# fragarriss/CurVis

Measured on AMD Instinct MI355X. Metric: Mrays/s (pixels x steps/s) at 1920x1080, 4096 steps, higher is better.
Workload: dtype f64

## Files before the change

curvis_amd/csrc/cv_sampler_dev.h:

```cpp
#ifndef CURVIS_CV_SAMPLER_DEV_H
#define CURVIS_CV_SAMPLER_DEV_H

#include "cv_math.h"

#if defined(__clang__)
#pragma clang fp contract(off)
#endif

namespace cvk {

constexpr unsigned kSamplerCap = 1536;
constexpr unsigned kSamplerPendCap = 1024;

enum : int { SAMPLER_OK = 0, SAMPLER_PANIC = 1, SAMPLER_OVERFLOW = 2 };

struct SamplerResult {
  unsigned n, rounds;
  unsigned long long calls, steps;
  int warned, status;
  unsigned eval_phases, evaluated;
};

constexpr unsigned kSpecSlots = 8192;
constexpr unsigned kSpecEvalCap = 2048;
constexpr unsigned kSpecEvalSoft = 1024;
constexpr unsigned long long kSpecEmpty = ~0ull;

struct SpecTable {
  unsigned long long *key;
  double *e, *s;
  unsigned *steps;
  int *status;
};

#if defined(__HIP_DEVICE_COMPILE__)
#define CV_SPEC_CAS(p, expect, val) atomicCAS((p), (expect), (val))
#define CV_SPEC_LD(p) __hip_atomic_load((p), __ATOMIC_RELAXED, __HIP_MEMORY_SCOPE_AGENT)
#define CV_SPEC_ST(p, v) __hip_atomic_store((p), (v), __ATOMIC_RELAXED, __HIP_MEMORY_SCOPE_AGENT)
#else
static inline unsigned long long cv_spec_cas_host(unsigned long long *p, unsigned long long expect, unsigned long long val) {
  const unsigned long long old = *p;
  if (old == expect) *p = val;
  return old;
}
#define CV_SPEC_CAS(p, expect, val) cv_spec_cas_host((p), (expect), (val))
#define CV_SPEC_LD(p) (*(p))
#define CV_SPEC_ST(p, v) (*(p) = (v))
#endif

CV_HD unsigned long long spec_key(double a) {
  unsigned long long k;
  __builtin_memcpy(&k, &a, sizeof k);
  return k;
}
CV_HD unsigned spec_hash(unsigned long long k) { return (unsigned)((k * 0x9E3779B97F4A7C15ull) >> 44) & (kSpecSlots - 1u); }
CV_HD unsigned spec_claim(const SpecTable &T, unsigned long long k, bool &fresh) {
  unsigned i = spec_hash(k);
  for (;;) {
    const unsigned long long old = CV_SPEC_CAS(&T.key[i], kSpecEmpty, k);
    if (old == kSpecEmpty) {
      fresh = true;
      return i;
    }
    if (old == k) {
      fresh = false;
      return i;
    }
    i = (i + 1u) & (kSpecSlots - 1u);
  }
}
CV_HD int spec_find(const SpecTable &T, unsigned long long k) {
  unsigned i = spec_hash(k);
  for (;;) {
    const unsigned long long cur = CV_SPEC_LD(&T.key[i]);
    if (cur == k) return (int)i;
    if (cur == kSpecEmpty) return -1;
    i = (i + 1u) & (kSpecSlots - 1u);
  }
}

CV_HD bool sampler_refine(double a1, double e1, double s1, double a2, double e2, double s2, double a3, double e3, double s3,
                          double thr1, double thr2) {
  const double area1 = CV_FABS((a1 * e2 + a2 * e3 + a3 * e1) - (e1 * a2 + e2 * a3 + e3 * a1));
  const double area2 = CV_FABS((a1 * s2 + a2 * s3 + a3 * s1) - (s1 * a2 + s2 * a3 + s3 * a1));
  return area1 > thr1 || area2 > thr2;
}
CV_HD bool sampler_finite(double v) { return (v - v) == 0.0; }

struct SamplerState {
  double a[2][kSamplerCap], e[2][kSamplerCap], s[2][kSamplerCap];
  double pend_a[kSamplerPendCap];
  unsigned short pend_out[kSamplerPendCap];
  unsigned char flag[kSamplerCap];
  unsigned short vis[kSamplerCap], vis_out[kSamplerCap];
  unsigned cur, n, n_new, n_pend, n_vis, iteration, prev_amount, rounds;
  int started, finished, panicked, warned, overflow, go, nonfinite;
  unsigned long long calls, steps;
  unsigned short miss[kSamplerPendCap];
  double eval_a[kSpecEvalCap];
  unsigned short eval_slot[kSpecEvalCap];
  unsigned n_miss, n_eval, n_cached , eval_phases, evaluated;
};

CV_HD void sampler_reset(SamplerState &S) {
  S.cur = S.n = S.n_new = S.n_pend = S.n_vis = S.iteration = S.prev_amount = S.rounds = 0u;
  S.started = S.finished = S.panicked = S.warned = S.overflow = S.go = S.nonfinite = 0;
  S.calls = S.steps = 0ull;
  S.n_miss = S.n_eval = S.n_cached = S.eval_phases = S.evaluated = 0u;
}


#if defined(__HIP_DEVICE_COMPILE__)
#define CV_LDS_INC(p) atomicAdd((p), 1u)
#define CV_LDS_ADD64(p, v) atomicAdd((p), (unsigned long long)(v))
#else
#define CV_LDS_INC(p) ((*(p))++)
#define CV_LDS_ADD64(p, v) (*(p) += (unsigned long long)(v))
#endif
struct SamplerState;
CV_HD void sampler_store(SamplerState &S, unsigned t, double e, double s);

CV_HD void sampler_finish(SamplerState &S, unsigned max_iterations) {
  if (S.iteration == max_iterations) S.warned = 1;
  S.finished = 1;
}

enum : int { PLAN_STOP = 0, PLAN_GRID = 1, PLAN_REFINE = 2 };

CV_HD int sampler_plan_begin(SamplerState &S, unsigned n0, unsigned max_iterations) {
  S.n_pend = 0u;
  if (S.finished) return PLAN_STOP;
  if (!S.started) {
    if (n0 > kSamplerCap || n0 > kSamplerPendCap) {
      S.overflow = S.finished = 1;
      return PLAN_STOP;
    }
    S.n_pend = S.n_new = n0;
    return PLAN_GRID;
  }
  if (!(S.iteration < max_iterations)) {
    sampler_finish(S, max_iterations);
    return PLAN_STOP;
  }
  S.prev_amount = S.n;
  if (S.n < 3u) {
    S.panicked = S.finished = 1;
    return PLAN_STOP;
  }
  return PLAN_REFINE;
}
CV_HD void sampler_grid_point(SamplerState &S, unsigned i, unsigned n0, double a_min, double a_max) {
  const double step = (a_max - a_min) / (double)(n0 - 1u);
  S.pend_a[i] = a_min + (double)i * step;
  S.pend_out[i] = (unsigned short)i;
}
CV_HD void sampler_flag(SamplerState &S, unsigned i, double thr1, double thr2) {
  const double *A = S.a[S.cur], *E = S.e[S.cur], *Z = S.s[S.cur];
  S.flag[i] = sampler_refine(A[i], E[i], Z[i], A[i + 1u], E[i + 1u], Z[i + 1u], A[i + 2u], E[i + 2u], Z[i + 2u], thr1, thr2) ? 1 : 0;
}
CV_HD bool sampler_walk(SamplerState &S) {
  const unsigned n = S.n;
  unsigned i = 0u, out = 0u, k = 0u, v = 0u;
  while (i < n - 2u) {
    if (out + 5u > kSamplerCap || k + 2u > kSamplerPendCap) {
      S.overflow = S.finished = 1;
      return false;
    }
    const unsigned f = S.flag[i];
    S.vis[v] = (unsigned short)(i | (f << 15));
    S.vis_out[v] = (unsigned short)out;
    ++v;
    if (f) {
      out += 4u, k += 2u, i += 2u;
    } else {
      out += 1u, i += 1u;
    }
  }
  S.n_vis = v;
  S.n_new = out;
  S.n_pend = k;
  return true;
}
CV_HD void sampler_place(SamplerState &S, unsigned v) {
  const unsigned dst = S.cur ^ 1u;
  const double *A = S.a[S.cur], *E = S.e[S.cur], *Z = S.s[S.cur];
  double *NA = S.a[dst], *NE = S.e[dst], *NZ = S.s[dst];
  const unsigned i = S.vis[v] & 0x7fffu, out = S.vis_out[v];
  NA[out] = A[i], NE[out] = E[i], NZ[out] = Z[i];
  if (S.vis[v] >> 15) {
    const unsigned k = 2u * ((out - v) / 3u);
    S.pend_a[k] = (A[i] + A[i + 1u]) / 2.0;
    S.pend_out[k] = (unsigned short)(out + 1u);
    NA[out + 2u] = A[i + 1u], NE[out + 2u] = E[i + 1u], NZ[out + 2u] = Z[i + 1u];
    S.pend_a[k + 1u] = (A[i + 1u] + A[i + 2u]) / 2.0;
    S.pend_out[k + 1u] = (unsigned short)(out + 3u);
    NA[out + 4u] = A[i + 2u], NE[out + 4u] = E[i + 2u], NZ[out + 4u] = Z[i + 2u];
  }
}
CV_HD bool sampler_plan(SamplerState &S, unsigned n0, unsigned max_iterations, double a_min, double a_max, double thr1, double thr2) {
  const int mode = sampler_plan_begin(S, n0, max_iterations);
  if (mode == PLAN_STOP) return false;
  if (mode == PLAN_GRID) {
    for (unsigned i = 0; i < n0; ++i) sampler_grid_point(S, i, n0, a_min, a_max);
    return true;
  }
  for (unsigned i = 0; i + 2u < S.n; ++i) sampler_flag(S, i, thr1, thr2);
  if (!sampler_walk(S)) return false;
  for (unsigned v = 0; v < S.n_vis; ++v) sampler_place(S, v);
  return true;
}

CV_HD void sampler_store(SamplerState &S, unsigned t, double e, double s) {
  const unsigned dst = S.cur ^ 1u, o = S.pend_out[t];
  S.a[dst][o] = S.pend_a[t];
  S.e[dst][o] = e;
  S.s[dst][o] = s;
  if (!(sampler_finite(e) && sampler_finite(s))) S.nonfinite = 1;
}

CV_HD bool sampler_take(SamplerState &S, const SpecTable &T, unsigned t, int &panic) {
  const int slot = spec_find(T, spec_key(S.pend_a[t]));
  if (slot < 0) return false;
  sampler_store(S, t, CV_SPEC_LD(&T.e[slot]), CV_SPEC_LD(&T.s[slot]));
  CV_LDS_ADD64(&S.steps, CV_SPEC_LD(&T.steps[slot]));
  if (CV_SPEC_LD(&T.status[slot]) == -2) panic = 1;
  return true;
}
CV_HD bool sampler_want(SamplerState &S, const SpecTable &T, double alpha, bool must) {
  if (!must && (S.n_cached >= kSpecSlots / 2u || S.n_eval >= kSpecEvalSoft)) return false;
  if (S.n_cached >= kSpecSlots - 1024u || S.n_eval >= kSpecEvalCap - 512u) {
    if (must) S.overflow = 1;
    return false;
  }
  bool fresh;
  const unsigned slot = spec_claim(T, spec_key(alpha), fresh);
  if (!fresh) return true;
  CV_LDS_INC(&S.n_cached);
  const unsigned k = CV_LDS_INC(&S.n_eval);
  S.eval_a[k] = alpha;
  S.eval_slot[k] = (unsigned short)slot;
  return true;
}
CV_HD void sampler_subtree(SamplerState &S, const SpecTable &T, double lo, double hi, unsigned depth) {
  if (depth > 7u) depth = 7u;
  for (unsigned level = 0u; level < depth; ++level)
    for (unsigned i = 0u; i < (1u << level); ++i) {
      double a = lo, b = hi, mid = (a + b) / 2.0;
      bool ok = mid > a && mid < b;
      for (unsigned bit = level; ok && bit-- > 0u;) {
        if ((i >> bit) & 1u)
          a = mid;
        else
          b = mid;
        mid = (a + b) / 2.0;
        ok = mid > a && mid < b;
      }
      if (ok && !sampler_want(S, T, mid, false)) return;
    }
}
CV_HD unsigned sampler_spec_depth(unsigned n, unsigned budget) {
  unsigned d = 0u;
  while (d < 7u && (unsigned long long)n * ((2ull << d) - 1ull) <= budget) ++d;
  return d;
}
CV_HD void sampler_speculate(SamplerState &S, const SpecTable &T, unsigned m, unsigned depth, unsigned grid_depth) {
  const unsigned t = S.miss[m];
  if (!S.started) {
    if (grid_depth && t + 1u < S.n_pend) sampler_subtree(S, T, S.pend_a[t], S.pend_a[t + 1u], grid_depth);
    return;
  }
  const unsigned dst = S.cur ^ 1u, o = S.pend_out[t];
  if (depth > 1u) {
    sampler_subtree(S, T, S.a[dst][o - 1u], S.pend_a[t], depth - 1u);
    sampler_subtree(S, T, S.pend_a[t], S.a[dst][o + 1u], depth - 1u);
  }
}

CV_HD void sampler_consume(SamplerState &S, unsigned max_iterations) {
  S.calls += S.n_pend;
  const unsigned dst = S.cur ^ 1u;
  double *NA = S.a[dst], *NE = S.e[dst], *NZ = S.s[dst];
  unsigned k = S.n_new;
  if (S.nonfinite) {
    k = 0u;
    for (unsigned i = 0; i < S.n_new; ++i)
      if (sampler_finite(NA[i]) && sampler_finite(NE[i]) && sampler_finite(NZ[i])) {
        if (k != i) NA[k] = NA[i], NE[k] = NE[i], NZ[k] = NZ[i];
        ++k;
      }
    S.nonfinite = 0;
  }
  S.n = k;
  S.cur = dst;
  if (!S.started) {
    S.started = 1;
    return;
  }
  S.rounds++;
  if (S.n <= S.prev_amount) {
    sampler_finish(S, max_iterations);
    return;
  }
  S.iteration += 1u;
}

}
#endif
```

curvis_amd/csrc/efficient_host.h:

```cpp
#pragma once

namespace {


struct EfficientCall {
  const curvis_metric *metric;
  const curvis_camera *cams;
  uint32_t n_frames, max_iter;
  double max_radius, delta;
  uint32_t alpha_nums, max_iterations_sampling;
  double thr1, thr2;
  uint32_t filter = 0;
  uint32_t ss = 1;
};

int eval_escape_batch(curvis_ctx *ctx, const curvis_metric *metric, const cvk::MetricParams &MP,
                      const std::vector<double> &alpha, const std::vector<double> &lcam, uint32_t max_iter,
                      double max_radius, double delta, std::vector<double> &angle, std::vector<double> &space,
                      std::vector<uint32_t> &steps, std::vector<int> &status, double *ms_acc) {
  const size_t n = alpha.size();
  angle.resize(n);
  space.resize(n);
  steps.resize(n);
  status.resize(n);
// ... 117 lines not shown
template <typename SampleMs>
void efficient_statistics(curvis_ctx *ctx, uint32_t n_frames, size_t npix, const FrameCounters &FC, SampleMs sample_ms, float pixel_ms,
                          curvis_stats *stats, std::chrono::steady_clock::time_point t_begin) {
  uint64_t tot[FC_N] = {0}, total_steps = 0;
  ctx->last_frame_stats.assign(n_frames, curvis_stats{});
  for (uint32_t f = 0; f < n_frames; ++f) {
    uint64_t fc[FC_N];
    sum_frame_counters(ctx->h_counters, FC.slots, f, fc);
    for (int k = 0; k < FC_N; ++k) tot[k] += fc[k];
    curvis_stats &fs = ctx->last_frame_stats[f];
    counts_to_stats(fc, fs);
    fs.rays = (uint64_t)npix;
    fs.steps = ctx->last_sampling_info[f].steps;
    total_steps += fs.steps;
    fs.integrate_ms = sample_ms / n_frames;
    fs.shade_ms = pixel_ms / n_frames;
    fs.kernel_ms = fs.integrate_ms + fs.shade_ms;
    fs.total_ms = fs.kernel_ms;
  }
  if (stats) {
    counts_to_stats(tot, *stats);
    stats->rays = (uint64_t)npix * n_frames;
    stats->steps = total_steps;
    stats->integrate_ms = sample_ms;
    stats->shade_ms = pixel_ms;
    stats->kernel_ms = sample_ms + pixel_ms;
    stats->total_ms = std::chrono::duration<double, std::milli>(std::chrono::steady_clock::now() - t_begin).count();
  }
}

constexpr int kSamplerFallback = 1;

curvis_ctx::SamplerKey make_sampler_key(const curvis_ctx *ctx, const EfficientCall &c) {
  curvis_ctx::SamplerKey k;
  k.metric = *c.metric;
  k.n_frames = c.n_frames;
  k.max_iter = c.max_iter;
  k.alpha_nums = c.alpha_nums;
  k.max_iterations_sampling = c.max_iterations_sampling;
  k.max_radius = c.max_radius, k.delta = c.delta, k.thr1 = c.thr1, k.thr2 = c.thr2;
  k.fast = ctx->fast_math != 0 ? 1 : 0;
  k.speculate = ctx->sampling_speculation != 0 ? 1 : 0;
  k.l_frame.resize(c.n_frames);
  for (uint32_t f = 0; f < c.n_frames; ++f) k.l_frame[f] = c.cams[f].pos[1];
  return k;
}
bool sampler_key_equal(const curvis_ctx::SamplerKey &a, const curvis_ctx::SamplerKey &b) {
  auto same = [](const double &x, const double &y) { return std::memcmp(&x, &y, sizeof(double)) == 0; };
  if (a.metric.kind != b.metric.kind || !same(a.metric.rho, b.metric.rho) || !same(a.metric.m, b.metric.m) || !same(a.metric.a, b.metric.a))
    return false;
  if (a.n_frames != b.n_frames || a.max_iter != b.max_iter || a.alpha_nums != b.alpha_nums ||
      a.max_iterations_sampling != b.max_iterations_sampling || a.fast != b.fast || a.speculate != b.speculate)
    return false;
  if (!same(a.max_radius, b.max_radius) || !same(a.delta, b.delta) || !same(a.thr1, b.thr1) || !same(a.thr2, b.thr2)) return false;
  return a.l_frame.size() == b.l_frame.size() &&
         std::memcmp(a.l_frame.data(), b.l_frame.data(), sizeof(double) * a.l_frame.size()) == 0;
}

int sampler_submit(curvis_ctx *ctx, unsigned slot, hipStream_t stream, const EfficientCall &c, const cvk::MetricParams &MP) {
  const curvis_camera *cams = c.cams;
  const uint32_t n_frames = c.n_frames;
  curvis_ctx::SamplerSlot &S = ctx->samp[slot];
  if (S.seq != 0 && S.done) HIP_TRY(ctx, hipEventSynchronize(S.done));
  if (ctx->dev_samples.valid && ctx->dev_samples.slot == slot) ctx->dev_samples.overwritten = true;
  S.valid = false;
  S.job_of_frame.assign(n_frames, 0u);
  S.l_job.clear();
  {
    std::map<uint64_t, unsigned> seen;
    for (uint32_t f = 0; f < n_frames; ++f) {
      uint64_t key;
      std::memcpy(&key, &cams[f].pos[1], sizeof key);
      auto it = seen.find(key);
      if (it == seen.end()) {
        it = seen.emplace(key, (unsigned)S.l_job.size()).first;
        S.l_job.push_back(cams[f].pos[1]);
      }
      S.job_of_frame[f] = it->second;
    }
  }
  const unsigned n_jobs = (unsigned)S.l_job.size();
  const size_t T = (size_t)n_jobs * cvk::kSamplerCap, SS = (size_t)n_jobs * cvk::kSpecSlots;
  size_t off = 0;
  auto carve = [&](size_t bytes) {
    const size_t o = off;
    off += (bytes + 255) & ~(size_t)255;
    return o;
  };
  const size_t o_jf = carve(sizeof(unsigned) * n_frames), o_to = carve(sizeof(unsigned) * n_frames), o_go = carve(sizeof(unsigned) * n_frames),
               o_l = carve(sizeof(double) * n_jobs);
  const size_t staged = off;
  S.o_tab_off = o_to;
  S.o_grid_off = o_go;
  S.o_grid = carve(sizeof(unsigned) * n_jobs * (cvk::kInterpGrid + 1u));
  S.o_tab_n = carve(sizeof(unsigned) * n_frames);
  S.o_res = carve(sizeof(cvk::SamplerResult) * n_jobs);
  for (size_t &o : S.o_tab) o = carve(sizeof(double) * T);
  const size_t o_sk = carve(sizeof(unsigned long long) * SS), o_se = carve(sizeof(double) * SS), o_ss = carve(sizeof(double) * SS),
               o_st = carve(sizeof(unsigned) * SS), o_su = carve(sizeof(int) * SS);
  int rc = S.d.reserve(ctx, off);
  if (rc) return rc;
  S.res_bytes = sizeof(cvk::SamplerResult) * n_jobs;
  S.h_res_off = staged;
  const size_t pinned = staged + ((S.res_bytes + 255) & ~(size_t)255);
  if ((rc = S.h.reserve(ctx, pinned, pinned / 2))) return rc;
  if ((rc = S.done.ensure(ctx, hipEventDisableTiming))) return rc;
  if ((rc = S.t0.ensure(ctx))) return rc;
  if ((rc = S.t1.ensure(ctx))) return rc;
  std::memcpy(S.h + o_jf, S.job_of_frame.data(), sizeof(unsigned) * n_frames);
  {
    auto *to = reinterpret_cast<unsigned *>(S.h + o_to);
    auto *go = reinterpret_cast<unsigned *>(S.h + o_go);
    for (uint32_t f = 0; f < n_frames; ++f) {
      to[f] = S.job_of_frame[f] * cvk::kSamplerCap;
      go[f] = S.job_of_frame[f] * (cvk::kInterpGrid + 1u);
    }
  }
  std::memcpy(S.h + o_l, S.l_job.data(), sizeof(double) * n_jobs);
  HIP_TRY(ctx, hipMemcpyAsync(S.d, S.h, staged, hipMemcpyHostToDevice, stream));
  HIP_TRY(ctx, hipMemsetAsync(S.d + o_sk, 0xFF, sizeof(unsigned long long) * SS, stream));
  curvis_ctx::SamplerKey key = make_sampler_key(ctx, c);
  SamplerParams SP;
  SP.metric = MP;
  SP.l_cam = (const double *)(S.d + o_l);
  SP.n_jobs = n_jobs;
  SP.n_frames = n_frames;
  SP.job_of_frame = (const unsigned *)(S.d + o_jf);
  SP.tab_n = (unsigned *)(S.d + S.o_tab_n);
  SP.n0 = c.alpha_nums;
  SP.max_iterations = c.max_iterations_sampling;
  SP.max_iter = c.max_iter;
  SP.a_min = -0.1 * CV_PI;
  SP.a_max = 1.1 * CV_PI;
  SP.thr1 = c.thr1;
  SP.thr2 = c.thr2;
  SP.max_radius = c.max_radius;
  SP.delta = c.delta;
  SP.fast_ok = cvk::metric_fast_ok(c.metric->kind, MP, c.max_radius) ? 1 : 0;
  SP.sx = (double *)(S.d + S.o_tab[0]);
  SP.se = (double *)(S.d + S.o_tab[1]);
  SP.ss = (double *)(S.d + S.o_tab[2]);
  SP.m_e = (double *)(S.d + S.o_tab[3]);
  SP.c_e = (double *)(S.d + S.o_tab[4]);
  SP.m_s = (double *)(S.d + S.o_tab[5]);
  SP.c_s = (double *)(S.d + S.o_tab[6]);
  SP.grid = (unsigned *)(S.d + S.o_grid);
  SP.res = (cvk::SamplerResult *)(S.d + S.o_res);
  SP.spec_key = (unsigned long long *)(S.d + o_sk);
  SP.spec_e = (double *)(S.d + o_se);
  SP.spec_s = (double *)(S.d + o_ss);
  SP.spec_steps = (unsigned *)(S.d + o_st);
  SP.spec_status = (int *)(S.d + o_su);
  SP.speculate = key.speculate;
  HIP_TRY(ctx, hipEventRecord(S.t0, stream));
  with_kind(c.metric->kind, [&](auto K) {
    with_flag(key.fast != 0, [&](auto F) {
      hipLaunchKernelGGL((sampler_kernel<decltype(K)::value, decltype(F)::value>), dim3(SP.n_jobs), dim3(kSamplerThreads), 0, stream, SP);
    });
  });
  HIP_TRY(ctx, hipGetLastError());
  HIP_TRY(ctx, hipEventRecord(S.t1, stream));
  HIP_TRY(ctx, hipMemcpyAsync(S.h + S.h_res_off, S.d + S.o_res, S.res_bytes, hipMemcpyDeviceToHost, stream));
  HIP_TRY(ctx, hipEventRecord(S.done, stream));
  S.key = std::move(key);
  S.seq = ++ctx->samp_seq;
  S.valid = true;
  return CURVIS_OK;
}

int prefetch_efficient_impl(curvis_ctx *ctx, const EfficientCall &c) {
  if (!ctx) return CURVIS_E_INVALID;
  if (!c.metric || !c.cams || c.n_frames == 0) return fail(ctx, CURVIS_E_INVALID, "null metric/camera or zero frames");
  int rc = curvis_metric_validate(c.metric);
  if (rc != CURVIS_OK) return fail(ctx, rc, "invalid metric parameters (src/metrics.rs:409-456)");
  if (c.alpha_nums < 3 || c.alpha_nums > cvk::kSamplerCap || c.alpha_nums > cvk::kSamplerPendCap) return CURVIS_OK;
  if (!(ctx->device_sampler > 0 || (ctx->device_sampler < 0 && c.n_frames >= (uint32_t)ctx->device_sampler_min_frames)))
    return CURVIS_OK;
  for (uint32_t f = 0; f < c.n_frames; ++f)
    if (std::fabs(c.cams[f].pos[1]) > c.max_radius) return CURVIS_OK;
  HIP_TRY(ctx, hipSetDevice(ctx->device));
  if ((rc = ctx->sampler_stream.ensure(ctx, hipStreamNonBlocking))) return rc;
  const unsigned slot = ctx->samp_next;
  rc = sampler_submit(ctx, slot, ctx->sampler_stream, c, make_metric(*c.metric));
  if (rc) return rc;
  ctx->samp[slot].prefetched = true;
  ctx->samp_next = slot ^ 1u;
  ctx->prefetches++;
  return CURVIS_OK;
}

int acquire_sampler_slot(curvis_ctx *ctx, const EfficientCall &c, const cvk::MetricParams &MP, int &slot, bool &prefetched) {
  const curvis_ctx::SamplerKey key = make_sampler_key(ctx, c);
  slot = -1;
  for (unsigned k = 0; k < 2u; ++k)
    if (ctx->samp[k].valid && ctx->samp[k].prefetched && sampler_key_equal(ctx->samp[k].key, key) &&
        (slot < 0 || ctx->samp[k].seq < ctx->samp[slot].seq))
      slot = (int)k;
  prefetched = slot >= 0;
  if (!prefetched) {
    slot = (int)ctx->samp_next;
    const int rc = sampler_submit(ctx, (unsigned)slot, ctx->stream, c, MP);
    if (rc) return rc;
    ctx->samp_next = (unsigned)slot ^ 1u;
  } else {
    HIP_TRY(ctx, hipStreamWaitEvent(ctx->stream, ctx->samp[slot].done, 0));
    ctx->prefetch_hits++;
  }
  ctx->samp[slot].prefetched = false;
  return CURVIS_OK;
}

void record_device_sampling(curvis_ctx *ctx, const curvis_ctx::SamplerSlot &S, const cvk::SamplerResult *h_res, uint32_t n_frames,
                            unsigned slot, bool prefetched, bool panic) {
  ctx->last_sampling_launches = 1;
  ctx->last_sampling_prefetched = prefetched ? 1 : 0;
  ctx->last_samples.assign(n_frames, {});
  ctx->last_sampling_info.assign(n_frames, curvis_sampling_info{});
  for (uint32_t f = 0; f < n_frames; ++f) {
    const cvk::SamplerResult &r = h_res[S.job_of_frame[f]];
    curvis_sampling_info &si = ctx->last_sampling_info[f];
    si.n_samples = r.n;
    si.rounds = r.rounds;
    si.calls = r.calls;
    si.steps = r.steps;
    si.warned_max_iterations = r.warned;
  }
  uint64_t evaluated = 0;
  uint32_t chains = 0;
  for (size_t j = 0; j < S.l_job.size(); ++j) {
    evaluated += h_res[j].evaluated;
    chains = std::max(chains, h_res[j].eval_phases);
  }
  ctx->last_sampling_evaluated = evaluated;
  ctx->last_sampling_chains = chains;
  ctx->dev_samples.valid = !panic;
  ctx->dev_samples.overwritten = false;
  ctx->dev_samples.slot = slot;
}

int render_efficient_device(curvis_ctx *ctx, const EfficientCall &c, const cvk::MetricParams &MP, const std::vector<cvk::EfficientFrame> &eframes,
                            uint8_t *rgb_out, curvis_stats *stats, std::chrono::steady_clock::time_point t_begin) {
  const uint32_t n_frames = c.n_frames, W = c.cams[0].res_x, H = c.cams[0].res_y;
  const size_t npix = (size_t)W * H;
  if (npix > 0xFFFFFFFFull || n_frames > 65535u) return fail(ctx, CURVIS_E_INVALID, "frame or batch too large");
  int slot = -1;
  bool prefetched = false;
  int rc = acquire_sampler_slot(ctx, c, MP, slot, prefetched);
  if (rc) return rc;
  curvis_ctx::SamplerSlot &S = ctx->samp[slot];
  const unsigned n_jobs = (unsigned)S.l_job.size();
  size_t off = 0;
  auto carve = [&](size_t bytes) {
    const size_t o = off;
    off += (bytes + 255) & ~(size_t)255;
    return o;
  };
  const size_t o_cams = carve(sizeof(cvk::CameraParams) * n_frames), o_fr = carve(sizeof(cvk::EfficientFrame) * n_frames);
  if ((rc = ctx->d_eff.reserve(ctx, off))) return rc;
  if ((rc = ctx->h_eff.reserve(ctx, off, off / 2))) return rc;
  unsigned char *stage = ctx->h_eff;
  {
    auto *cp = reinterpret_cast<cvk::CameraParams *>(stage + o_cams);
    for (uint32_t f = 0; f < n_frames; ++f) cp[f] = make_camera(c.cams[f]);
    std::memcpy(stage + o_fr, eframes.data(), sizeof(cvk::EfficientFrame) * n_frames);
  }
  const size_t fb_bytes = (size_t)(W / c.ss) * (H / c.ss) * 3 * n_frames;
  rc = fb_begin_write(ctx, fb_bytes);
  if (rc) return rc;
  ctx->fb_bytes = fb_bytes;
  HIP_TRY(ctx, hipMemcpyAsync(ctx->d_eff, stage, off, hipMemcpyHostToDevice, ctx->stream));
  HIP_TRY(ctx, hipEventRecord(ctx->ev1, ctx->stream));
  FrameCounters FC;
  rc = prepare_counters(ctx, n_frames, FC, 64u);
  if (rc) return rc;
  const size_t cnt_words = counter_words(n_frames, FC.slots);
  EfficientPixelParams Q;
  const PixelInputs in = {ctx->d_eff, o_cams, o_fr, S.d, S.o_tab_off, S.o_tab_n, S.o_grid_off, S.o_grid, S.o_tab[0], S.o_tab[3],
                          S.o_tab[4], S.o_tab[5], S.o_tab[6]};
  if ((rc = make_pixel_params(ctx, n_frames, W, H, FC, in, Q))) return rc;
  if ((rc = launch_pixel_kernel(ctx, Q, n_frames, c.ss, c.filter))) return rc;
  HIP_TRY(ctx, hipEventRecord(ctx->ev2, ctx->stream));
  HIP_TRY(ctx, hipMemcpyAsync(ctx->h_counters, ctx->d_counters, sizeof(unsigned long long) * cnt_words, hipMemcpyDeviceToHost, ctx->stream));
  const auto t_launched = std::chrono::steady_clock::now();
  HIP_TRY(ctx, hipStreamSynchronize(ctx->stream));
  if (getenv("CURVIS_DEBUG_TIMING")) {
    float k_ms = 0.f;
    (void)hipEventElapsedTime(&k_ms, ctx->ev1, ctx->ev2);
    const auto t_now = std::chrono::steady_clock::now();
    fprintf(stderr, "[curvis] efficient call, %u frames (ms): host before the sync %.3f, in the sync %.3f (staging copy -> end of the per-pixel kernel: %.3f)\n",
            n_frames, std::chrono::duration<double, std::milli>(t_launched - t_begin).count(),
            std::chrono::duration<double, std::milli>(t_now - t_launched).count(), k_ms);
  }
  auto *h_res = reinterpret_cast<const cvk::SamplerResult *>(S.h + S.h_res_off);
  bool overflow = false, panic = false;
  for (unsigned j = 0; j < n_jobs; ++j) {
    overflow = overflow || h_res[j].status == cvk::SAMPLER_OVERFLOW;
    panic = panic || h_res[j].status == cvk::SAMPLER_PANIC;
  }
  if (getenv("CURVIS_DEBUG_TIMING"))
    for (unsigned j = 0; j < n_jobs; ++j)
      fprintf(stderr, "[curvis] device sampler job %u: l = %.17g -> %u samples, %u rounds, %llu calls, %llu steps, warned %d, status %d; "
              "%u Euler chains, %u points integrated%s\n", j, S.l_job[j], h_res[j].n, h_res[j].rounds, (unsigned long long)h_res[j].calls,
              (unsigned long long)h_res[j].steps, h_res[j].warned, h_res[j].status, h_res[j].eval_phases, h_res[j].evaluated,
              prefetched ? " (prefetched)" : "");
  if (overflow) return kSamplerFallback;
  float sample_ms = 0.f, ms = 0.f;
  HIP_TRY(ctx, hipEventElapsedTime(&sample_ms, S.t0, S.t1));
  HIP_TRY(ctx, hipEventElapsedTime(&ms, ctx->ev1, ctx->ev2));
  record_device_sampling(ctx, S, h_res, n_frames, (unsigned)slot, prefetched, panic);
  if (panic)
    return fail(ctx, CURVIS_E_SAMPLING,
                "sampler panic: fewer than 3 finite samples (src/sampling.rs:155-157) or undefined tangent rotation "
                "(src/algebra.rs:95-97)");
  if (rgb_out) {
// ... 462 lines not shown
```

curvis_amd/csrc/kernels_efficient.h:

```cpp
#pragma once

namespace {


struct EscapeAngleParams {
  cvk::MetricParams metric;
  const double *alpha;
  const double *l_cam;
  double *angle;
  double *space;
  unsigned *steps;
  int *status;
  unsigned n;
  unsigned max_iter;
  double max_radius, delta;
  int fast_ok;
};

template <int KIND, bool FAST>
__device__ __forceinline__ void escape_angle_lane(const cvk::MetricParams &M, double alpha, double l_cam, unsigned max_iter, double max_radius,
                                                  double delta, int fast_ok, double &angle, double &space, unsigned &steps_out, int &status) {
  double sa, ca;
  cv_sincos(alpha, &sa, &ca);
  const double pos[4] = {0.0, l_cam, CV_PI / 2.0, 0.0};
  cvk::Ray q;
  cvk::ray_init_dir<KIND>(M, pos, ca, 0.0, sa, q);
  const bool lane_ok = FAST && fast_ok && cvk::ray_fast_ok(q);
  unsigned steps = max_iter;
  int code = cvk::CODE_NONE;
  if (max_iter != 0) {
    const unsigned lane = threadIdx.x & 63u;
    unsigned k = 0;
    for (;;) {
      ++k;
      one_step<KIND, true, FAST, true>(M, delta, q, lane_ok);
      const bool esc = ray_escaped(q.l, max_radius);
      const unsigned long long em = __builtin_amdgcn_ballot_w64(esc);
      if (em) {
        unsigned kv;
        asm volatile("v_mov_b32 %0, %1" : "=v"(kv) : "s"(k));
        if ((em >> lane) & 1ull) steps = kv;
      }
      if (esc) break;
      if (k >= max_iter) break;
    }
    if (ray_escaped(q.l, max_radius)) code = escape_code(q.l);
  } else {
    steps = 0;
  }
  const double nan = __builtin_nan("");
  angle = nan;
  space = nan;
  status = code;
  if (code != cvk::CODE_NONE) {
    if (cvk::escape_angle_of<KIND>(M, q, angle)) {
      space = (code == cvk::CODE_POS) ? 1.0 : -1.0;
    } else {
      angle = nan;
      status = cvk::ESC_PANIC;
    }
  }
  steps_out = steps;
}

template <int KIND, bool FAST>
__global__ __launch_bounds__(64) void escape_angle_kernel(const EscapeAngleParams P) {
  __shared__ MathTablesLds<KIND> s_tab;
  cvk::MetricParams M = P.metric;
  load_math_tables<KIND>(s_tab, M);
  const unsigned i = blockIdx.x * blockDim.x + threadIdx.x;
  if (i >= P.n) return;
  double angle, space;
  unsigned steps;
  int status;
  escape_angle_lane<KIND, FAST>(M, P.alpha[i], P.l_cam[i], P.max_iter, P.max_radius, P.delta, P.fast_ok, angle, space, steps, status);
  P.angle[i] = angle;
  P.space[i] = space;
  P.steps[i] = steps;
  P.status[i] = status;
}

struct SamplerParams {
  cvk::MetricParams metric;
  const double *l_cam;
  unsigned n_jobs, n_frames;
  const unsigned *job_of_frame;
  unsigned *tab_n;
  unsigned n0, max_iterations, max_iter;
  double a_min, a_max, thr1, thr2, max_radius, delta;
  int fast_ok;
  double *sx, *se, *ss, *m_e, *c_e, *m_s, *c_s;
  unsigned *grid;
  cvk::SamplerResult *res;
  unsigned long long *spec_key;
  double *spec_e, *spec_s;
  unsigned *spec_steps;
  int *spec_status;
  int speculate;
};
constexpr unsigned kSamplerThreads = 512;

template <int KIND, bool FAST>
__global__ __launch_bounds__(kSamplerThreads) void sampler_kernel(const SamplerParams P) {
  __shared__ MathTablesLds<KIND> s_tab;
  __shared__ cvk::SamplerState S;
  __shared__ int s_panic;
  cvk::MetricParams M = P.metric;
  if (threadIdx.x == 0u) {
    cvk::sampler_reset(S);
    s_panic = 0;
  }
  load_math_tables<KIND>(s_tab, M);
  const unsigned job = blockIdx.x;
  const double l_cam = P.l_cam[job];
  cvk::SpecTable T;
  {
    const size_t so = (size_t)job * cvk::kSpecSlots;
    T.key = P.spec_key + so;
    T.e = P.spec_e + so;
    T.s = P.spec_s + so;
    T.steps = P.spec_steps + so;
    T.status = P.spec_status + so;
  }
  for (;;) {
    if (threadIdx.x == 0u) {
      S.go = cvk::sampler_plan_begin(S, P.n0, P.max_iterations);
      S.n_miss = S.n_eval = 0u;
    }
    __syncthreads();
    const int mode = S.go;
    if (mode == cvk::PLAN_STOP) break;
    if (mode == cvk::PLAN_GRID) {
      for (unsigned i = threadIdx.x; i < P.n0; i += kSamplerThreads) cvk::sampler_grid_point(S, i, P.n0, P.a_min, P.a_max);
    } else {
      for (unsigned i = threadIdx.x; i + 2u < S.n; i += kSamplerThreads) cvk::sampler_flag(S, i, P.thr1, P.thr2);
      __syncthreads();
      if (threadIdx.x == 0u) S.go = cvk::sampler_walk(S) ? cvk::PLAN_REFINE : cvk::PLAN_STOP;
      __syncthreads();
      if (S.go == cvk::PLAN_STOP) break;
      for (unsigned v = threadIdx.x; v < S.n_vis; v += kSamplerThreads) cvk::sampler_place(S, v);
    }
    __syncthreads();
    const unsigned np = S.n_pend;
    for (unsigned t = threadIdx.x; t < np; t += kSamplerThreads) {
      int panic = 0;
      if (!cvk::sampler_take(S, T, t, panic)) S.miss[atomicAdd(&S.n_miss, 1u)] = (unsigned short)t;
      if (panic) s_panic = 1;
    }
    __syncthreads();
    const unsigned nm = S.n_miss;
    if (nm) {
      for (unsigned m = threadIdx.x; m < nm; m += kSamplerThreads) cvk::sampler_want(S, T, S.pend_a[S.miss[m]], true);
      __syncthreads();
      if (P.speculate && !S.overflow) {
        const unsigned depth = S.started ? cvk::sampler_spec_depth(nm, kSamplerThreads) : 0u;
        const unsigned grid_depth = (!S.started && kSamplerThreads > nm) ? cvk::sampler_spec_depth(nm - 1u, kSamplerThreads - nm) : 0u;
        for (unsigned m = threadIdx.x; m < nm; m += kSamplerThreads) cvk::sampler_speculate(S, T, m, depth, grid_depth);
      }
      __syncthreads();
      const unsigned ne = S.n_eval < cvk::kSpecEvalCap ? S.n_eval : cvk::kSpecEvalCap;
      for (unsigned base = 0; base < ne; base += kSamplerThreads) {
        const unsigned k = base + threadIdx.x;
        if (k < ne) {
          double angle, space;
          unsigned steps;
          int status;
          escape_angle_lane<KIND, FAST>(M, S.eval_a[k], l_cam, P.max_iter, P.max_radius, P.delta, P.fast_ok, angle, space, steps, status);
          const unsigned slot = S.eval_slot[k];
          CV_SPEC_ST(&T.e[slot], angle);
          CV_SPEC_ST(&T.s[slot], space);
          CV_SPEC_ST(&T.steps[slot], steps);
          CV_SPEC_ST(&T.status[slot], status);
        }
      }
      if (threadIdx.x == 0u) {
        S.eval_phases += (ne + kSamplerThreads - 1u) / kSamplerThreads;
        S.evaluated += ne;
      }
      __syncthreads();
      for (unsigned m = threadIdx.x; m < nm; m += kSamplerThreads) {
        int panic = 0;
        if (!cvk::sampler_take(S, T, S.miss[m], panic)) S.overflow = 1;
        if (panic) s_panic = 1;
      }
      __syncthreads();
    }
    if (threadIdx.x == 0u) {
      if (S.overflow) S.finished = 1;
      cvk::sampler_consume(S, P.max_iterations);
    }
    __syncthreads();
  }
  const unsigned n = S.n, cur = S.cur;
  const size_t o = (size_t)job * cvk::kSamplerCap;
  const double *A = S.a[cur], *E = S.e[cur], *Z = S.s[cur];
  const unsigned slots = n ? n : 1u;
  for (unsigned i = threadIdx.x; i < slots; i += kSamplerThreads) {
    const bool have = i < n;
    P.sx[o + i] = have ? A[i] : 0.0;
    P.se[o + i] = have ? E[i] : 0.0;
    P.ss[o + i] = have ? Z[i] : 0.0;
    double me = 0.0, ce = 0.0, ms = 0.0, cs = 0.0;
    if (n == 1u) {
      ce = E[0];
      cs = Z[0];
    } else if (i + 1u < n) {
      const double dx = A[i + 1u] - A[i];
      me = (E[i + 1u] - E[i]) / dx;
      ce = E[i] - A[i] * me;
      ms = (Z[i + 1u] - Z[i]) / dx;
      cs = Z[i] - A[i] * ms;
    }
    P.m_e[o + i] = me;
    P.c_e[o + i] = ce;
    P.m_s[o + i] = ms;
    P.c_s[o + i] = cs;
  }
  for (unsigned i = threadIdx.x; i <= n; i += kSamplerThreads) cvk::interp_grid_fill(A, n, i, P.grid + (size_t)job * (cvk::kInterpGrid + 1u));
  for (unsigned f = threadIdx.x; f < P.n_frames; f += kSamplerThreads)
    if (P.job_of_frame[f] == job) P.tab_n[f] = n;
  if (threadIdx.x == 0u) {
    cvk::SamplerResult r;
    r.n = n;
    r.rounds = S.rounds;
    r.calls = S.calls;
    r.steps = S.steps;
    r.warned = S.warned;
    r.status = S.overflow ? cvk::SAMPLER_OVERFLOW : (S.panicked || s_panic) ? cvk::SAMPLER_PANIC : cvk::SAMPLER_OK;
    r.eval_phases = S.eval_phases;
    r.evaluated = S.evaluated;
    P.res[job] = r;
  }
}

struct EfficientPixelParams {
  cvk::SkyParams sky[2];
  const cvk::CameraParams *cams;
  const cvk::EfficientFrame *frames;
  const unsigned *tab_off;
  const unsigned *tab_n;
  const unsigned *grid_off;
  const unsigned *grid;
  const double *sx, *m_e, *c_e, *m_s, *c_s;
  unsigned n_frames, W, H;
  unsigned char *fb;
  FrameCounters counters;
  cvk::PixelRecips recips;
  unsigned long long w_magic;
};

__global__ void recip_chain_kernel(const double *d, double *y, unsigned n) {
  if (threadIdx.x < n) y[threadIdx.x] = cvk::recip_chain(d[threadIdx.x]);
}

template <int FILTER = 0>
__global__ __launch_bounds__(256) void efficient_pixel_kernel(const EfficientPixelParams P) {
  __shared__ __attribute__((aligned(16))) unsigned char s_rgb[256 * 3];
  __shared__ unsigned s_cnt[5];
  const unsigned f = blockIdx.y;
  const unsigned npix = P.W * P.H;
  const unsigned pix = blockIdx.x * 256u + threadIdx.x;
  const bool valid = pix < npix;
  if (threadIdx.x < 5u) s_cnt[threadIdx.x] = 0u;
  bool pos = false, neg = false, none = false, oob = false;
  unsigned texel = 0xFF000000u;
  if (valid) {
    const unsigned py = P.w_magic ? (unsigned)__umul64hi((unsigned long long)pix, P.w_magic) : pix / P.W, px = pix - py * P.W;
    const unsigned off = P.tab_off[f], n = P.tab_n[f];
    double fin[3], space;
    cvk::efficient_pixel<true>(P.cams[f], P.frames[f], px, py, P.sx + off, P.m_e + off, P.c_e + off, P.m_s + off, P.c_s + off, n, fin, space,
                               &P.recips, P.grid + P.grid_off[f]);
    pos = (space == 1.0);
    neg = (space == -1.0);
    none = !(pos || neg);
#pragma unroll
    for (int k = 0; k < 2; ++k) {
      if (k == 0 ? pos : neg) {
        const cvk::SkyParams &S = P.sky[k];
        unsigned tx, ty;
        if constexpr (FILTER != 0) {
          if (sky_lookup_bilinear<true>(S, fin[0], fin[1], fin[2], tx, ty, texel, P.recips.y_pi, P.recips.y_two_pi)) oob = true;
        } else {
          cvk::sky_indices<true>(S, fin[0], fin[1], fin[2], tx, ty, P.recips.y_pi, P.recips.y_two_pi);
          if (tx >= S.w || ty >= S.h) oob = true;
          if (tx >= S.w) tx = S.w - 1;
          if (ty >= S.h) ty = S.h - 1;
          texel = S.texels[(size_t)ty * S.w + tx];
        }
      }
    }
  }
  unsigned char *fb = P.fb + (size_t)f * npix * 3u;
  const unsigned lane = threadIdx.x & 63u, wave = threadIdx.x >> 6;
  const unsigned long long vm = __builtin_amdgcn_ballot_w64(valid);
  if (vm == ~0ull && ((((size_t)f * npix * 3u) & 3u) == 0u)) {
    unsigned char *sw = s_rgb + wave * 192u;
    sw[3u * lane + 0u] = (unsigned char)(texel & 0xFF);
    sw[3u * lane + 1u] = (unsigned char)((texel >> 8) & 0xFF);
    sw[3u * lane + 2u] = (unsigned char)((texel >> 16) & 0xFF);
    __builtin_amdgcn_wave_barrier();
    if (lane < 48u) reinterpret_cast<unsigned *>(fb + (size_t)(pix - lane) * 3u)[lane] = reinterpret_cast<const unsigned *>(sw)[lane];
  } else if (valid) {
    store_rgb8(fb + (size_t)pix * 3u, texel);
  }
  const unsigned n_pos = (unsigned)__popcll(__builtin_amdgcn_ballot_w64(pos)), n_neg = (unsigned)__popcll(__builtin_amdgcn_ballot_w64(neg));
  const unsigned n_none = (unsigned)__popcll(__builtin_amdgcn_ballot_w64(none)), n_oob = (unsigned)__popcll(__builtin_amdgcn_ballot_w64(oob));
  __syncthreads();
  if (lane == 0u && vm) {
    atomicAdd(&s_cnt[0], (unsigned)__popcll(vm));
    if (n_pos) atomicAdd(&s_cnt[1], n_pos);
    if (n_neg) atomicAdd(&s_cnt[2], n_neg);
    if (n_none) atomicAdd(&s_cnt[3], n_none);
    if (n_oob) atomicAdd(&s_cnt[4], n_oob);
  }
  __syncthreads();
  if (threadIdx.x == 0u && s_cnt[0]) {
    unsigned long long *c = frame_counter_line(P.counters, f);
    atomicAdd(&c[FC_RAYS], (unsigned long long)s_cnt[0]);
    if (s_cnt[1]) atomicAdd(&c[FC_POS], (unsigned long long)s_cnt[1]);
    if (s_cnt[2]) atomicAdd(&c[FC_NEG], (unsigned long long)s_cnt[2]);
    if (s_cnt[3]) atomicAdd(&c[FC_NONE], (unsigned long long)s_cnt[3]);
    if (s_cnt[4]) atomicAdd(&c[FC_OOB], (unsigned long long)s_cnt[4]);
  }
}

template <int SS, int FILTER = 0>
__global__ __launch_bounds__(256) void efficient_pixel_ss_kernel(const EfficientPixelParams P) {
  __shared__ unsigned s_cnt[5];
  const unsigned f = blockIdx.y;
  const unsigned tiles_x = (P.W + 7u) >> 3;
  const unsigned lane = threadIdx.x & 63u, wave = threadIdx.x >> 6;
  const unsigned tile = blockIdx.x * 4u + wave;
  const unsigned tyi = tile / tiles_x, txi = tile - tyi * tiles_x;
  const unsigned px = txi * 8u + (lane & 7u), py = tyi * 8u + (lane >> 3);
  const bool valid = px < P.W && py < P.H;
  if (threadIdx.x < 5u) s_cnt[threadIdx.x] = 0u;
  bool pos = false, neg = false, none = false, oob = false;
  unsigned texel = 0xFF000000u;
  if (valid) {
    const unsigned off = P.tab_off[f], n = P.tab_n[f];
    double fin[3], space;
    cvk::efficient_pixel<true>(P.cams[f], P.frames[f], px, py, P.sx + off, P.m_e + off, P.c_e + off, P.m_s + off, P.c_s + off, n, fin, space,
                               &P.recips, P.grid + P.grid_off[f]);
    pos = (space == 1.0);
// ... 335 lines not shown
```

Before: 394,700.

## Parallelize sampler refinement walk with tree-based prefix scan across block lanes

```diff
diff --git a/curvis_amd/csrc/cv_sampler_dev.h b/curvis_amd/csrc/cv_sampler_dev.h
--- a/curvis_amd/csrc/cv_sampler_dev.h
+++ b/curvis_amd/csrc/cv_sampler_dev.h
@@ -11,6 +11,9 @@
 
 constexpr unsigned kSamplerCap = 1536;
 constexpr unsigned kSamplerPendCap = 1024;
+constexpr unsigned kSamplerLanes = 512;
+constexpr unsigned kWalkPerLane = kSamplerCap / kSamplerLanes;
+static_assert(kWalkPerLane * kSamplerLanes == kSamplerCap && kSamplerLanes == 8u * 8u * 8u, "sampler_walk_lane: three levels of eight");
 
 enum : int { SAMPLER_OK = 0, SAMPLER_PANIC = 1, SAMPLER_OVERFLOW = 2 };
 
@@ -93,6 +96,8 @@
   unsigned short pend_out[kSamplerPendCap];
   unsigned char flag[kSamplerCap];
   unsigned short vis[kSamplerCap], vis_out[kSamplerCap];
+  unsigned walk_tree[2][kSamplerLanes + 64u + 8u];
+  unsigned char walk_mask[kSamplerLanes];
   unsigned cur, n, n_new, n_pend, n_vis, iteration, prev_amount, rounds;
   int started, finished, panicked, warned, overflow, go, nonfinite;
   unsigned long long calls, steps;
@@ -158,11 +163,11 @@
   const double *A = S.a[S.cur], *E = S.e[S.cur], *Z = S.s[S.cur];
   S.flag[i] = sampler_refine(A[i], E[i], Z[i], A[i + 1u], E[i + 1u], Z[i + 1u], A[i + 2u], E[i + 2u], Z[i + 2u], thr1, thr2) ? 1 : 0;
 }
-CV_HD bool sampler_walk(SamplerState &S) {
+CV_HD bool sampler_walk(SamplerState &S, unsigned cap = kSamplerCap, unsigned pend_cap = kSamplerPendCap) {
   const unsigned n = S.n;
   unsigned i = 0u, out = 0u, k = 0u, v = 0u;
   while (i < n - 2u) {
-    if (out + 5u > kSamplerCap || k + 2u > kSamplerPendCap) {
+    if (out + 5u > cap || k + 2u > pend_cap) {
       S.overflow = S.finished = 1;
       return false;
     }
@@ -180,6 +185,98 @@
   S.n_new = out;
   S.n_pend = k;
   return true;
+}
+
+constexpr unsigned kWalkPhases = 7u;
+constexpr unsigned kWalkL1 = kSamplerLanes, kWalkL2 = kSamplerLanes + 64u;
+
+template <bool MAX>
+CV_HD unsigned walk_combine(unsigned a, unsigned b) {
+  if (MAX) return a > b ? a : b;
+  return a + b;
+}
+template <bool MAX>
+CV_HD void walk_reduce8(unsigned *tree, unsigned from, unsigned to, unsigned t) {
+  unsigned r = 0u;
+  for (unsigned j = 0u; j < 8u; ++j) r = walk_combine<MAX>(r, tree[from + 8u * t + j]);
+  tree[to + t] = r;
+}
+template <bool MAX>
+CV_HD unsigned walk_prefix(const unsigned *tree, unsigned t) {
+  unsigned r = 0u;
+  for (unsigned j = 0u; j < (t >> 6); ++j) r = walk_combine<MAX>(r, tree[kWalkL2 + j]);
+  for (unsigned j = 8u * (t >> 6); j < (t >> 3); ++j) r = walk_combine<MAX>(r, tree[kWalkL1 + j]);
+  for (unsigned j = 8u * (t >> 3); j < t; ++j) r = walk_combine<MAX>(r, tree[j]);
+  return r;
+}
+CV_HD void sampler_walk_lane(SamplerState &S, unsigned phase, unsigned t, unsigned cap = kSamplerCap, unsigned pend_cap = kSamplerPendCap) {
+  const unsigned nt = S.n - 2u, i0 = kWalkPerLane * t;
+  unsigned *mx = S.walk_tree[0], *sm = S.walk_tree[1];
+  switch (phase) {
+    case 0u: {
+      unsigned z = 0u;
+      for (unsigned j = 0u; j < kWalkPerLane; ++j)
+        if (i0 + j < nt && !S.flag[i0 + j]) z = i0 + j + 1u;
+      mx[t] = z;
+      break;
+    }
+    case 1u:
+      if (t < 64u) walk_reduce8<true>(mx, 0u, kWalkL1, t);
+      break;
+    case 2u:
+      if (t < 8u) walk_reduce8<true>(mx, kWalkL1, kWalkL2, t);
+      break;
+    case 3u: {
+      unsigned z = walk_prefix<true>(mx, t), mask = 0u, cv = 0u, cr = 0u;
+      for (unsigned j = 0u; j < kWalkPerLane; ++j) {
+        const unsigned i = i0 + j;
+        if (i < nt) {
+          const unsigned f = S.flag[i];
+          if (((i - z) & 1u) == 0u) mask |= 1u << j, cv += 1u, cr += f;
+          if (!f) z = i + 1u;
+        }
+      }
+      S.walk_mask[t] = (unsigned char)mask;
+      sm[t] = cv | (cr << 16);
+      break;
+    }
+    case 4u:
+      if (t < 64u) walk_reduce8<false>(sm, 0u, kWalkL1, t);
+      break;
+    case 5u:
+      if (t < 8u) walk_reduce8<false>(sm, kWalkL1, kWalkL2, t);
+      if (t == 0u) S.go = PLAN_REFINE;
+      break;
+    default: {
+      const unsigned p = walk_prefix<false>(sm, t), mask = S.walk_mask[t];
+      unsigned cv = p & 0xffffu, cr = p >> 16;
+      for (unsigned j = 0u; j < kWalkPerLane; ++j)
+        if ((mask >> j) & 1u) {
+          const unsigned i = i0 + j, f = S.flag[i], out = cv + 3u * cr;
+          if (out + 5u > cap || 2u * cr + 2u > pend_cap) {
+            S.overflow = S.finished = 1;
+            S.go = PLAN_STOP;
+          } else {
+            S.vis[cv] = (unsigned short)(i | (f << 15));
+            S.vis_out[cv] = (unsigned short)out;
+          }
+          cv += 1u, cr += f;
+        }
+      if (t == 0u) {
+        unsigned tot = 0u;
+        for (unsigned j = 0u; j < 8u; ++j) tot += sm[kWalkL2 + j];
+        S.n_vis = tot & 0xffffu;
+        S.n_new = (tot & 0xffffu) + 3u * (tot >> 16);
+        S.n_pend = 2u * (tot >> 16);
+      }
+      break;
+    }
+  }
+}
+CV_HD bool sampler_walk_lanes(SamplerState &S, unsigned cap = kSamplerCap, unsigned pend_cap = kSamplerPendCap) {
+  for (unsigned phase = 0u; phase < kWalkPhases; ++phase)
+    for (unsigned t = 0u; t < kSamplerLanes; ++t) sampler_walk_lane(S, phase, t, cap, pend_cap);
+  return S.go == PLAN_REFINE;
 }
 CV_HD void sampler_place(SamplerState &S, unsigned v) {
   const unsigned dst = S.cur ^ 1u;
diff --git a/curvis_amd/csrc/efficient_host.h b/curvis_amd/csrc/efficient_host.h
--- a/curvis_amd/csrc/efficient_host.h
+++ b/curvis_amd/csrc/efficient_host.h
@@ -293,6 +293,14 @@
   SP.spec_steps = (unsigned *)(S.d + o_st);
   SP.spec_status = (int *)(S.d + o_su);
   SP.speculate = key.speculate;
+  DeviceBuffer<unsigned long long> trace;
+  const char *trace_file = getenv("CURVIS_TRACE_FILE");
+  const size_t trace_words = (size_t)n_jobs * kSamplerTraceRounds * 8u;
+  if (trace_file && *trace_file) {
+    if ((rc = trace.reserve(ctx, trace_words))) return rc;
+    HIP_TRY(ctx, hipMemsetAsync(trace, 0, trace_words * sizeof(unsigned long long), stream));
+  }
+  SP.trace = trace;
   HIP_TRY(ctx, hipEventRecord(S.t0, stream));
   with_kind(c.metric->kind, [&](auto K) {
     with_flag(key.fast != 0, [&](auto F) {
@@ -301,6 +309,15 @@
   });
   HIP_TRY(ctx, hipGetLastError());
   HIP_TRY(ctx, hipEventRecord(S.t1, stream));
+  if (trace) {
+    std::vector<unsigned long long> tr(trace_words);
+    HIP_TRY(ctx, hipMemcpyAsync(tr.data(), trace, trace_words * sizeof(unsigned long long), hipMemcpyDeviceToHost, stream));
+    HIP_TRY(ctx, hipStreamSynchronize(stream));
+    if (FILE *fp = fopen(trace_file, "wb")) {
+      fwrite(tr.data(), sizeof(unsigned long long), tr.size(), fp);
+      fclose(fp);
+    }
+  }
   HIP_TRY(ctx, hipMemcpyAsync(S.h + S.h_res_off, S.d + S.o_res, S.res_bytes, hipMemcpyDeviceToHost, stream));
   HIP_TRY(ctx, hipEventRecord(S.done, stream));
   S.key = std::move(key);
diff --git a/curvis_amd/csrc/kernels_efficient.h b/curvis_amd/csrc/kernels_efficient.h
--- a/curvis_amd/csrc/kernels_efficient.h
+++ b/curvis_amd/csrc/kernels_efficient.h
@@ -97,8 +97,11 @@
   unsigned *spec_steps;
   int *spec_status;
   int speculate;
+  unsigned long long *trace;
 };
-constexpr unsigned kSamplerThreads = 512;
+constexpr unsigned kSamplerTraceRounds = 64;
+enum SamplerStamp : unsigned { ST_BEGIN = 0, ST_FLAGS, ST_WALK, ST_PLACE, ST_TAKE, ST_CHAIN, ST_END, ST_SIZES };
+constexpr unsigned kSamplerThreads = cvk::kSamplerLanes;
 
 template <int KIND, bool FAST>
 __global__ __launch_bounds__(kSamplerThreads) void sampler_kernel(const SamplerParams P) {
@@ -122,7 +125,13 @@
     T.steps = P.spec_steps + so;
     T.status = P.spec_status + so;
   }
-  for (;;) {
+  unsigned round = 0u;
+  unsigned long long *const trace = P.trace ? P.trace + (size_t)job * kSamplerTraceRounds * 8u : nullptr;
+  auto stamp = [&](unsigned which) {
+    if (trace && threadIdx.x == 0u && round < kSamplerTraceRounds) trace[round * 8u + which] = wall_clock64();
+  };
+  for (;; ++round) {
+    stamp(ST_BEGIN);
     if (threadIdx.x == 0u) {
       S.go = cvk::sampler_plan_begin(S, P.n0, P.max_iterations);
       S.n_miss = S.n_eval = 0u;
@@ -135,12 +144,23 @@
     } else {
       for (unsigned i = threadIdx.x; i + 2u < S.n; i += kSamplerThreads) cvk::sampler_flag(S, i, P.thr1, P.thr2);
       __syncthreads();
+      stamp(ST_FLAGS);
+#if defined(CV_SAMPLER_SERIAL_WALK)
       if (threadIdx.x == 0u) S.go = cvk::sampler_walk(S) ? cvk::PLAN_REFINE : cvk::PLAN_STOP;
       __syncthreads();
+#else
+#pragma unroll
+      for (unsigned phase = 0u; phase < cvk::kWalkPhases; ++phase) {
+        cvk::sampler_walk_lane(S, phase, threadIdx.x);
+        __syncthreads();
+      }
+#endif
+      stamp(ST_WALK);
       if (S.go == cvk::PLAN_STOP) break;
       for (unsigned v = threadIdx.x; v < S.n_vis; v += kSamplerThreads) cvk::sampler_place(S, v);
     }
     __syncthreads();
+    stamp(ST_PLACE);
     const unsigned np = S.n_pend;
     for (unsigned t = threadIdx.x; t < np; t += kSamplerThreads) {
       int panic = 0;
@@ -158,6 +178,7 @@
         for (unsigned m = threadIdx.x; m < nm; m += kSamplerThreads) cvk::sampler_speculate(S, T, m, depth, grid_depth);
       }
       __syncthreads();
+      stamp(ST_TAKE);
       const unsigned ne = S.n_eval < cvk::kSpecEvalCap ? S.n_eval : cvk::kSpecEvalCap;
       for (unsigned base = 0; base < ne; base += kSamplerThreads) {
         const unsigned k = base + threadIdx.x;
@@ -178,6 +199,7 @@
         S.evaluated += ne;
       }
       __syncthreads();
+      stamp(ST_CHAIN);
       for (unsigned m = threadIdx.x; m < nm; m += kSamplerThreads) {
         int panic = 0;
         if (!cvk::sampler_take(S, T, S.miss[m], panic)) S.overflow = 1;
@@ -185,11 +207,14 @@
       }
       __syncthreads();
     }
+    if (trace && threadIdx.x == 0u && round < kSamplerTraceRounds)
+      trace[round * 8u + ST_SIZES] = (unsigned long long)S.n | (unsigned long long)np << 16 | (unsigned long long)nm << 32 | (unsigned long long)S.n_eval << 48;
     if (threadIdx.x == 0u) {
       if (S.overflow) S.finished = 1;
       cvk::sampler_consume(S, P.max_iterations);
     }
     __syncthreads();
+    stamp(ST_END);
   }
   const unsigned n = S.n, cur = S.cur;
   const size_t o = (size_t)job * cvk::kSamplerCap;
```

After: 396,000 (median of 3 runs). About the same (+0.3%).
